# YessionCC/AR-NeRF

Measured on AMD Instinct MI355X. Metric: training rays/sec + test PSNR, Lego 8192-ray batch, 1/2/4/8 MI355X, higher is better.
Workload: dtype fp16 field (MLP forward, backward and weight gradients on fp16 MFMA operands, fp32 accumulate) / fp32 march, composite, Adam; 1 GPU; lego-shaped training step: 8192 rays/rank, scale 0.5, 1 x 128^3 grid, L=16 F=2 T=2^19 hash, 64-wide MLPs, raw loss, Adam lr 1e-2; batch_rays_per_gpu=8192, global_batch_rays=8192, pretrain_steps=2000, graphs=True, chunk_first=64, row_forward=1, march_fork=r1, parallelism=dp1, hash_backward=hybrid, bin_level_lo=8, bin_merge_hi=11, steps_per_graph_replay=2, erode=False

## Files before the change

### ar-nerf_amd/csrc/field.hip

```cpp
#pragma clang fp contract(off)

#include <algorithm>

#include "common.h"
#include "field_net.h"
#include "grid.h"
#include "transmittance.h"

namespace ngp {

struct __attribute__((aligned(4))) u2a4 {
    uint32_t x, y;
    __device__ operator uint2() const { return make_uint2(x, y); }
};

__device__ __forceinline__ uint32_t pick4(uint4 q, uint32_t k) {
    return k == 0 ? q.x : k == 1 ? q.y : k == 2 ? q.z : q.w;
}

__device__ __forceinline__ void fetch_pair(const uint32_t* __restrict__ tl, uint32_t i0, uint32_t i1, bool dense,
                                           uint32_t& v0, uint32_t& v1) {
    const uint32_t lo = min(i0, i1), hi = max(i0, i1);
    uint32_t vlo, vhi;
    if (dense) {
// ... 90 lines not shown
    uint32_t pg[3];
    level_cell(in, u, pg, pos);
    gather_cell(pg, u, table, v);
}
__device__ __forceinline__ uint32_t level_sum_h2(const float in[3], const LevelU& u, const uint32_t v[8]) {
    float pos[3], w[8];
    uint32_t pg[3];
    level_cell(in, u, pg, pos);
    corner_weights(pos, w);
    float a0, a1;
    sum_level(w, v, a0, a1);
    return pack_h2(a0, a1);
}

__device__ __forceinline__ void encode_level(const float in[3], const LevelU& u, const uint32_t* __restrict__ table,
                                             float& a0, float& a1) {
    float pos[3], w[8];
    uint32_t pg[3], v[8];
    level_cell(in, u, pg, pos);
    corner_weights(pos, w);
#pragma unroll
    for (int yz = 0; yz < 4; ++yz) {
        uint32_t i0, i1;
        pair_index(pg, yz, u, i0, i1);
        fetch_pair(table + u.off, i0, i1, u.dense || !u.pow2, v[2 * yz], v[2 * yz + 1]);
    }
    sum_level(w, v, a0, a1);
}

__device__ __forceinline__ h8 encode4(const float in[3], int g, const LevelLds& lv, const uint32_t* __restrict__ table) {
    h8 e;
#pragma unroll
    for (int jl = 0; jl < 4; ++jl) {
        float a0, a1;
        encode_level(in, level_lane(lv, 4 * g + jl), table, a0, a1);
        e[2 * jl] = (_Float16)a0;
        e[2 * jl + 1] = (_Float16)a1;
    }
    return e;
}


template <bool COLOR, bool ENC_IN = false>
__global__ void __launch_bounds__(256) field_fwd_kernel(const float* __restrict__ xyzs, const float* __restrict__ dirs,
                                                        int64_t n, const int64_t* __restrict__ n_dev, GridArgs ga,
                                                        const uint32_t* __restrict__ table,
                                                        const _Float16* __restrict__ mlp, float* __restrict__ sigmas,
                                                        float* __restrict__ rgbs, _Float16* __restrict__ enc_out,
                                                        _Float16* __restrict__ h_out,
                                                        const _Float16* __restrict__ enc_in = nullptr,
                                                        int64_t enc_stride = 0,
                                                        const int32_t* __restrict__ sidx = nullptr,
                                                        int act = NGP_RGB_SIGMOID) {
    __shared__ __attribute__((aligned(16))) _Float16 sw[SWF];
    __shared__ LevelLds lv;
    load_fwd_weights_direct(mlp, sw, COLOR);
    if constexpr (!ENC_IN) load_levels(ga, lv);
    __syncthreads();
    const int64_t N = ngp_capped_count(n_dev, n);
    const int lane = threadIdx.x & 63, s = lane & 15, g = lane >> 4;
    const int64_t nw = (int64_t)gridDim.x * (blockDim.x >> 6);
    for (int64_t base = ((int64_t)blockIdx.x * (blockDim.x >> 6) + (threadIdx.x >> 6)) * 16; base < N; base += nw * 16) {
        const int64_t j = base + s;
        const bool valid = j < N;
        const int64_t i = valid && sidx ? (int64_t)sidx[j] : j;
        h8 e;
        if constexpr (ENC_IN) {
            const h4 z4 = {0, 0, 0, 0};
            const h4 ea = valid ? *reinterpret_cast<const h4*>(enc_in + ((2 * g) * enc_stride + i) * 4) : z4;
            const h4 eb = valid ? *reinterpret_cast<const h4*>(enc_in + ((2 * g + 1) * enc_stride + i) * 4) : z4;
            e = pack(ea, eb);
        } else {
            float in[3];
            load_x01(xyzs, i, valid, ga, in);
            e = encode4(in, g, lv, table);
        }
        h4 h1[4];
        const h4 hh = density_net(e, sw, s, g, h1);
        if (valid) {
            if (enc_out) *reinterpret_cast<h8*>(enc_out + i * 32 + 8 * g) = e;
            if (h_out) *reinterpret_cast<h4*>(h_out + i * 16 + 4 * g) = hh;
            if (g == 0) sigmas[i] = expf((float)hh[0]);
        }
        if constexpr (COLOR) {
            const float dx = valid ? dirs[3 * i] : 0.f, dy = valid ? dirs[3 * i + 1] : 0.f,
                        dz = valid ? dirs[3 * i + 2] : 1.f;
            float sh[4];
            sh4_select(dx, dy, dz, g, sh);
            const h8 cin = {(_Float16)sh[0], (_Float16)sh[1], (_Float16)sh[2], (_Float16)sh[3], hh[0], hh[1], hh[2], hh[3]};
            h4 h3[4], h4v[4];
            const h4 o = color_net(cin, sw, s, g, h3, h4v);
            if (valid && g == 0) {
                rgbs[3 * i] = rgb_out(o[0], act);
                rgbs[3 * i + 1] = rgb_out(o[1], act);
                rgbs[3 * i + 2] = rgb_out(o[2], act);
            }
        }
    }
}

__global__ void __launch_bounds__(256) hash_encode_kernel(const float* __restrict__ xyzs, int64_t n,
                                                          const int64_t* __restrict__ n_dev,
                                                          const int32_t* __restrict__ sidx, GridArgs ga,
                                                          const uint32_t* __restrict__ table,
                                                          _Float16* __restrict__ enc_pm) {
    __shared__ LevelLds lv;
    load_levels(ga, lv);
    __syncthreads();
    const int64_t N = ngp_capped_count(n_dev, n);
    for (int64_t j = (int64_t)blockIdx.x * blockDim.x + threadIdx.x; j < N; j += (int64_t)gridDim.x * blockDim.x) {
        const int64_t i = sidx ? (int64_t)sidx[j] : j;
        float in[3];
        load_x01(xyzs, i, true, ga, in);
#pragma unroll 1
        for (int pr = 0; pr < 8; ++pr) {
            float w[2][8];
            uint32_t v[2][8];
            gather_level_u(in, level_u(lv, 2 * pr), table, w[0], v[0]);
            gather_level_u(in, level_u(lv, 2 * pr + 1), table, w[1], v[1]);
            float a0, a1, b0, b1;
            sum_level(w[0], v[0], a0, a1);
            sum_level(w[1], v[1], b0, b1);
            *reinterpret_cast<h4*>(enc_pm + ((int64_t)pr * n + i) * 4) =
                h4{(_Float16)a0, (_Float16)a1, (_Float16)b0, (_Float16)b1};
        }
    }
}

__device__ __forceinline__ void transpose_rows4(uint32_t E[16]) {
#pragma unroll
    for (int k = 0; k < 4; ++k) {
        const auto a = __builtin_amdgcn_permlane32_swap(E[k], E[8 + k], false, false);
        E[k] = a[0];
        E[8 + k] = a[1];
        const auto b = __builtin_amdgcn_permlane32_swap(E[4 + k], E[12 + k], false, false);
        E[4 + k] = b[0];
        E[12 + k] = b[1];
    }
#pragma unroll
    for (int k = 0; k < 4; ++k) {
        const auto a = __builtin_amdgcn_permlane16_swap(E[k], E[4 + k], false, false);
        E[k] = a[0];
        E[4 + k] = a[1];
        const auto b = __builtin_amdgcn_permlane16_swap(E[8 + k], E[12 + k], false, false);
        E[8 + k] = b[0];
        E[12 + k] = b[1];
    }
}

constexpr int FEM2_WAVES = 8, FEM_LPR = 2;
constexpr int PRE_LEVELS = 8;
static_assert(PRE_LEVELS % FEM_LPR == 0 && PRE_LEVELS % 2 == 0, "pre-encoded levels: whole rounds and pairs");
static_assert(L % FEM_LPR == 0, "levels per round");
__device__ __forceinline__ void encode_rounds(const float in[3], const LevelLds& lv, const uint32_t* __restrict__ table,
                                              int r0, uint32_t E[16]) {
#pragma unroll 1
    for (int r = r0; r < L / FEM_LPR; ++r) {
        uint32_t v[FEM_LPR][8];
#pragma unroll
        for (int q = 0; q < FEM_LPR; ++q) gather_level_loads(in, level_u(lv, FEM_LPR * r + q), table, v[q]);
#pragma unroll
        for (int q = 0; q < 16 - FEM_LPR; ++q) E[q] = E[q + FEM_LPR];
#pragma unroll
        for (int q = 0; q < FEM_LPR; ++q) E[16 - FEM_LPR + q] = level_sum_h2(in, level_u(lv, FEM_LPR * r + q), v[q]);
    }
}
template <bool COLOR>
__global__ void __launch_bounds__(64 * FEM2_WAVES, FEM2_WAVES / 2) field_encode_mlp_reg_kernel(
    const float* __restrict__ xyzs, const float* __restrict__ dirs, int64_t n, const int64_t* __restrict__ n_dev,
    const int32_t* __restrict__ sidx, GridArgs ga, const uint32_t* __restrict__ table,
    const _Float16* __restrict__ mlp, _Float16* __restrict__ enc_pm, float* __restrict__ sigmas,
    float* __restrict__ rgbs, _Float16* __restrict__ h_out, int act) {
    __shared__ __attribute__((aligned(16))) _Float16 sw[SWF];
    __shared__ LevelLds lv;
    NGP_PROBE_BEGIN(NGP_P_FIELD_ENCODE_MLP);
    const int64_t N = ngp_capped_count(n_dev, n);
    const int lane = threadIdx.x & 63, wv = threadIdx.x >> 6;
    const int64_t G = gridDim.x;
    const int64_t chunks = (N + 63) >> 6;
    int64_t k = (int64_t)wv * G + blockIdx.x;
    int64_t i_first = 0;
    float in_first[3];
    {
        const int64_t j = k * 64 + lane;
        const bool valid = k < chunks && j < N;
        i_first = valid ? (sidx ? (int64_t)sidx[j] : j) : 0;
        load_x01(xyzs, i_first, valid, ga, in_first);
    }
    load_fwd_weights_direct(mlp, sw, COLOR);
    load_levels(ga, lv);
    __syncthreads();
    bool first = true;
    for (; k < chunks; k += (int64_t)FEM2_WAVES * G) {
        int lane_l = lane;
        asm volatile("" : "+v"(lane_l));
        const int s = lane_l & 15, g = lane_l >> 4;
        const int64_t j = k * 64 + lane_l;
        const bool valid = j < N;
        int64_t i = i_first;
        float in[3] = {in_first[0], in_first[1], in_first[2]};
        if (!first) {
            i = valid ? (sidx ? (int64_t)sidx[j] : j) : 0;
            load_x01(xyzs, i, valid, ga, in);
        }
        first = false;
        uint32_t E[16];
        encode_rounds(in, lv, table, 0, E);
        if (valid && enc_pm) {
#pragma unroll
            for (int pr = 0; pr < 8; ++pr)
                *reinterpret_cast<uint2*>(enc_pm + ((int64_t)pr * n + i) * 4) = make_uint2(E[2 * pr], E[2 * pr + 1]);
        }
        transpose_rows4(E);
        const int32_t imine = valid ? (int32_t)i : -1;
#pragma unroll 1
        for (int c = 0; c < 4; ++c) {
            const int32_t ic = __shfl(imine, 16 * c + s, 64);
            const bool ok = ic >= 0;
            const h8 e = __builtin_bit_cast(h8, make_uint4(E[0], E[1], E[2], E[3]));
#pragma unroll
            for (int q = 0; q < 12; ++q) E[q] = E[q + 4];
            h4 h1[4];
            const h4 hh = density_net(e, sw, s, g, h1);
            if (ok) {
                if (h_out) *reinterpret_cast<h4*>(h_out + (int64_t)ic * 16 + 4 * g) = hh;
                if (g == 0) sigmas[ic] = expf((float)hh[0]);
            }
            if constexpr (COLOR) {
                const float dx = ok ? dirs[3 * (int64_t)ic] : 0.f, dy = ok ? dirs[3 * (int64_t)ic + 1] : 0.f,
                            dz = ok ? dirs[3 * (int64_t)ic + 2] : 1.f;
                float sh[4];
                sh4_select(dx, dy, dz, g, sh);
                const h8 cin = {(_Float16)sh[0], (_Float16)sh[1], (_Float16)sh[2], (_Float16)sh[3], hh[0], hh[1], hh[2], hh[3]};
                h4 h3[4], h4v[4];
                const h4 o = color_net(cin, sw, s, g, h3, h4v);
                if (ok && g == 0) {
                    rgbs[3 * (int64_t)ic] = rgb_out(o[0], act);
                    rgbs[3 * (int64_t)ic + 1] = rgb_out(o[1], act);
                    rgbs[3 * (int64_t)ic + 2] = rgb_out(o[2], act);
                }
            }
        }
    }
    NGP_PROBE_END();
}

template <bool COLOR>
__device__ __forceinline__ float encode_mlp_chunk(const float* __restrict__ xyzs, const float* __restrict__ dirs,
                                                  int64_t i0, int cnt, int64_t n, const GridArgs& ga,
                                                  const LevelLds& lv, const uint32_t* __restrict__ table,
                                                  const _Float16* sw, _Float16* __restrict__ enc_pm,
                                                  float* __restrict__ sigmas, float* __restrict__ rgbs, int pre = 0,
                                                  int act = NGP_RGB_SIGMOID) {
    int lane_l = threadIdx.x & 63;
    asm volatile("" : "+v"(lane_l));
    const int s = lane_l & 15, g = lane_l >> 4;
    const bool valid = lane_l < cnt;
    const int64_t i = i0 + lane_l;
    float in[3];
    load_x01(xyzs, i, valid, ga, in);
    uint32_t E[16];
    if (pre) {
#pragma unroll
        for (int pr = 0; pr < PRE_LEVELS / 2; ++pr) {
            const uint2 q = valid ? *reinterpret_cast<const uint2*>(enc_pm + ((int64_t)pr * n + i) * 4) : make_uint2(0u, 0u);
            E[16 - PRE_LEVELS + 2 * pr] = q.x;
            E[16 - PRE_LEVELS + 2 * pr + 1] = q.y;
        }
    }
    encode_rounds(in, lv, table, pre / FEM_LPR, E);
    if (valid && enc_pm) {
#pragma unroll
        for (int pr = 0; pr < 8; ++pr)
            if (2 * pr >= pre)
                *reinterpret_cast<uint2*>(enc_pm + ((int64_t)pr * n + i) * 4) = make_uint2(E[2 * pr], E[2 * pr + 1]);
    }
    transpose_rows4(E);
    float sg = 0.f;
#pragma unroll 1
    for (int c = 0; c < 4; ++c) {
        if (16 * c >= cnt) break;
        const bool ok = 16 * c + s < cnt;
        const int64_t ic = i0 + 16 * c + s;
        const h8 e = __builtin_bit_cast(h8, make_uint4(E[0], E[1], E[2], E[3]));
#pragma unroll
        for (int q = 0; q < 12; ++q) E[q] = E[q + 4];
        h4 h1[4];
        const h4 hh = density_net(e, sw, s, g, h1);
        const float sig = expf((float)hh[0]);
        if (ok && g == 0) sigmas[ic] = sig;
        const float sgc = __shfl(sig, lane_l & 15, 64);
        if ((lane_l >> 4) == c) sg = sgc;
        if constexpr (COLOR) {
            const float dx = ok ? dirs[3 * ic] : 0.f, dy = ok ? dirs[3 * ic + 1] : 0.f, dz = ok ? dirs[3 * ic + 2] : 1.f;
            float sh[4];
            sh4_select(dx, dy, dz, g, sh);
            const h8 cin = {(_Float16)sh[0], (_Float16)sh[1], (_Float16)sh[2], (_Float16)sh[3], hh[0], hh[1], hh[2], hh[3]};
            h4 h3[4], h4v[4];
            const h4 o = color_net(cin, sw, s, g, h3, h4v);
            if (ok && g == 0) {
                rgbs[3 * ic] = rgb_out(o[0], act);
                rgbs[3 * ic + 1] = rgb_out(o[1], act);
                rgbs[3 * ic + 2] = rgb_out(o[2], act);
            }
        }
    }
    return sg;
}

template <bool COLOR>
__global__ void __launch_bounds__(64 * FEM2_WAVES, FEM2_WAVES / 2) field_first_chunk_kernel(
    const float* __restrict__ xyzs, const float* __restrict__ dirs, const float* __restrict__ deltas,
    const int64_t* __restrict__ rays_a, const int32_t* __restrict__ rows, const int64_t* __restrict__ n_rows_dev,
    int64_t n_rows, int64_t n, float T_thr, GridArgs ga, const uint32_t* __restrict__ table,
    const _Float16* __restrict__ mlp, _Float16* __restrict__ enc_pm, float* __restrict__ sigmas,
    float* __restrict__ rgbs, int32_t* __restrict__ rest, int32_t* __restrict__ list2, int64_t* __restrict__ total2,
    int64_t* __restrict__ evaluated, int pre, int act) {
    __shared__ __attribute__((aligned(16))) _Float16 sw[SWF];
    __shared__ LevelLds lv;
    __shared__ unsigned long long blk_eval;
    NGP_PROBE_BEGIN(NGP_P_FIRST_CHUNK);
    const int lane = threadIdx.x & 63, wv = threadIdx.x >> 6;
    const int64_t NR = ngp_capped_count(n_rows_dev, n_rows);
    const int64_t G = gridDim.x, stride = (int64_t)FEM2_WAVES * G;
    int64_t j = (int64_t)wv * G + blockIdx.x;
    int64_t r = 0, start = 0, N = 0;
    if (j < NR) {
        r = rows ? (int64_t)rows[j] : j;
        start = rays_a[3 * r + 1];
        N = rays_a[3 * r + 2];
    }
    if (threadIdx.x == 0) blk_eval = 0ull;
    load_fwd_weights_direct(mlp, sw, COLOR);
    load_levels(ga, lv);
    __syncthreads();
    int64_t ev = 0;
    for (; j < NR; j += stride) {
        const int cnt = (int)(N < 64 ? N : 64);
        int32_t rc = 0;
        if (cnt > 0) {
            const float dl = lane < cnt ? deltas[start + lane] : 0.f;
            const float sg = encode_mlp_chunk<COLOR>(xyzs, dirs, start, cnt, n, ga, lv, table, sw, enc_pm, sigmas, rgbs,
                                                     pre, act);
            const float om = 1.0f - (1.0f - __expf(-sg * dl));
            const ChunkT ct = chunk_transmittance(om, cnt, 1.0f, T_thr, lane);
            rc = (!ct.hit && N > 64) ? (int32_t)(N - 64) : 0;
            ev += cnt;
        }
        if (rest && lane == 0) rest[r] = rc;
        if (list2 && rc > 0) {
            unsigned long long o = 0;
            if (lane == 0) o = atomicAdd((unsigned long long*)total2, (unsigned long long)rc);
            const int64_t o2 = (int64_t)__shfl(o, 0, 64);
            if (lane == 0 && o2 + rc > n) ngp_guard_hit();
            for (int t = lane; t < rc && o2 + t < n; t += 64) list2[o2 + t] = (int32_t)(start + 64 + t);
            ev += rc;
        }
        const int64_t jn = j + stride;
        if (jn < NR) {
            r = rows ? (int64_t)rows[jn] : jn;
            start = rays_a[3 * r + 1];
            N = rays_a[3 * r + 2];
        }
    }
    if (lane == 0 && ev) atomicAdd(&blk_eval, (unsigned long long)ev);
    __syncthreads();
    if (threadIdx.x == 0 && evaluated && blk_eval) atomicAdd((unsigned long long*)evaluated, blk_eval);
    NGP_PROBE_END();
}

__global__ void __launch_bounds__(256) encode_coarse_first_kernel(
    const float* __restrict__ xyzs, const int64_t* __restrict__ rays_a, const int32_t* __restrict__ rows,
    const int64_t* __restrict__ n_rows_dev, int64_t n_rows, int64_t n, GridArgs ga,
    const uint32_t* __restrict__ table, _Float16* __restrict__ enc_pm) {
    __shared__ LevelLds lv;
    NGP_PROBE_BEGIN(NGP_P_PRE_ENCODE);
    load_levels(ga, lv);
    __syncthreads();
    const int lane = threadIdx.x & 63;
    const int64_t NR = ngp_capped_count(n_rows_dev, n_rows);
    constexpr int NP = PRE_LEVELS / 2;
    const int64_t stride = (int64_t)gridDim.x * (blockDim.x >> 6);
    for (int64_t q = (int64_t)blockIdx.x * (blockDim.x >> 6) + (threadIdx.x >> 6); q < NR * NP; q += stride) {
        const int64_t j = q / NP;
        const int pr = (int)(q - j * NP);
        const int64_t r = rows ? (int64_t)rows[j] : j;
        const int64_t start = rays_a[3 * r + 1], N = rays_a[3 * r + 2];
        const bool valid = lane < N;
        const int64_t i = start + lane;
        float in[3];
        load_x01(xyzs, i, valid, ga, in);
        uint32_t v[2][8];
        gather_level_loads(in, level_u(lv, 2 * pr), table, v[0]);
        gather_level_loads(in, level_u(lv, 2 * pr + 1), table, v[1]);
        const uint32_t e0 = level_sum_h2(in, level_u(lv, 2 * pr), v[0]);
        const uint32_t e1 = level_sum_h2(in, level_u(lv, 2 * pr + 1), v[1]);
        if (valid) *reinterpret_cast<uint2*>(enc_pm + ((int64_t)pr * n + i) * 4) = make_uint2(e0, e1);
    }
    NGP_PROBE_END();
}

__device__ __forceinline__ void coarse_level_runs(const float in[3], bool valid, float gd, int l, const LevelLds& lv,
                                                  int lane, int cx, uint32_t idx[4], float v[4], uint64_t heads[4]) {
    const float sc = lv.scale[l];
    const uint32_t res = lv.res[l], size = lv.size[l], off = lv.off[l];
    const bool dense = (lv.dense >> l) & 1u, pow2 = (lv.pow2 >> l) & 1u;
    float pos[3];
    uint32_t pg[3];
    level_cell(sc, in, pg, pos);
#pragma unroll
    for (int yz = 0; yz < 4; ++yz) {
        const int cy = yz & 1, cz = yz >> 1;
        float wt = 1.0f;
        wt *= cx ? pos[0] : 1 - pos[0];
        wt *= cy ? pos[1] : 1 - pos[1];
        wt *= cz ? pos[2] : 1 - pos[2];
        idx[yz] = valid ? off + corner_index(pg[0] + cx, pg[1] + cy, pg[2] + cz, res, size, dense, pow2)
                        : 0xffffffffu;
        v[yz] = wt * gd;
    }
    uint32_t prev[4];
#pragma unroll
    for (int yz = 0; yz < 4; ++yz) prev[yz] = __shfl_up(idx[yz], 4, 64);
#pragma unroll
    for (int yz = 0; yz < 4; ++yz) heads[yz] = __ballot(lane < 4 || prev[yz] != idx[yz]);
    if ((heads[0] & heads[1] & heads[2] & heads[3]) != ~0ull) {
#pragma unroll
        for (int o4 = 4; o4 < 64; o4 <<= 1) {
            float ov[4];
#pragma unroll
            for (int yz = 0; yz < 4; ++yz) ov[yz] = __shfl_down(v[yz], o4, 64);
            const uint64_t span = ((0x1111111111111111ull & ((2ull << o4) - 1ull)) & ~1ull) << lane;
#pragma unroll
            for (int yz = 0; yz < 4; ++yz)
                if (lane + o4 < 64 && (heads[yz] & span) == 0) v[yz] += ov[yz];
        }
    }
}

__device__ __forceinline__ void coarse_scatter_level(const float in[3], bool valid, float gd, int l, const LevelLds& lv,
                                                     float* __restrict__ dst, int lane, int cx, int f) {
    uint32_t idx[4];
    float v[4];
    uint64_t heads[4];
    coarse_level_runs(in, valid, gd, l, lv, lane, cx, idx, v, heads);
#pragma unroll
    for (int yz = 0; yz < 4; ++yz) {
        const bool head = (heads[yz] >> lane) & 1ull;
        if (head && valid) atomicAdd(&dst[2 * (size_t)idx[yz] + f], v[yz]);
    }
}

typedef _Float16 h2v __attribute__((ext_vector_type(2)));
__device__ __forceinline__ f4 mfma16(h4 a, h4 b, f4 c) { return __builtin_amdgcn_mfma_f32_16x16x16f16(a, b, c, 0, 0, 0); }
__device__ __forceinline__ h4 lds4(const _Float16* p) { return *reinterpret_cast<const h4*>(p); }

constexpr int RT16 = 20, RT64 = 68;
constexpr int BT5 = SWF, BT4 = BT5 + 64 * RT16, BT3 = BT4 + 64 * RT64, BT2 = BT3 + 16 * RT64, BT1 = BT2 + 64 * RT16,
              BTE = BT1 + 32 * RT64;
constexpr int TROW = 16, TTILE = 16 * TROW;
constexpr int SCR = (BTE + 7) & ~7;

__device__ __forceinline__ void load_bwd_weights(const _Float16* __restrict__ mlp, _Float16* sw) {
    const int t = threadIdx.x, nt = blockDim.x;
    for (int e = t; e < 64 * 16; e += nt) { const int i = e >> 4, o = e & 15; sw[BT5 + i * RT16 + o] = mlp[OW5 + o * 64 + i]; }
    for (int e = t; e < 64 * 64; e += nt) { const int i = e >> 6, o = e & 63; sw[BT4 + i * RT64 + o] = mlp[OW4 + o * 64 + i]; }
    for (int e = t; e < 16 * 64; e += nt) { const int i = e >> 6, o = e & 63; sw[BT3 + i * RT64 + o] = mlp[OW3 + o * 32 + 16 + i]; }
    for (int e = t; e < 64 * 16; e += nt) { const int i = e >> 4, o = e & 15; sw[BT2 + i * RT16 + o] = mlp[OW2 + o * 64 + i]; }
    for (int e = t; e < 32 * 64; e += nt) { const int i = e >> 6, o = e & 63; sw[BT1 + i * RT64 + o] = mlp[OW1 + o * 32 + i]; }
}

__device__ __forceinline__ void load_bwd_weights_direct(const _Float16* __restrict__ mlp, _Float16* sw) {
    constexpr int N1 = 128, N2 = 64, N3 = 128, N4 = 256, N5 = 64, NI = N1 + N2 + N3 + N4 + N5;
    for (int it = threadIdx.x; it < NI; it += blockDim.x) {
        int ow, lg_cb, li, bt, rt, skip;
        if (it < N1) { ow = OW1; lg_cb = 2; li = it; bt = BT1; rt = RT64; skip = 0; }
        else if (it < N1 + N2) { ow = OW2; lg_cb = 3; li = it - N1; bt = BT2; rt = RT16; skip = 0; }
        else if (it < N1 + N2 + N3) { ow = OW3; lg_cb = 2; li = it - N1 - N2; bt = BT3; rt = RT64; skip = 16; }
        else if (it < NI - N5) { ow = OW4; lg_cb = 3; li = it - N1 - N2 - N3; bt = BT4; rt = RT64; skip = 0; }
        else { ow = OW5; lg_cb = 3; li = it - (NI - N5); bt = BT5; rt = RT16; skip = 0; }
        const int in_dim = 8 << lg_cb, o = 2 * (li >> lg_cb), i0 = 8 * (li & ((1 << lg_cb) - 1));
        const int f0 = ow + o * in_dim + i0;
        const h8 a = *reinterpret_cast<const h8*>(mlp + f0);
        const h8 b = *reinterpret_cast<const h8*>(mlp + f0 + in_dim);
        place_fwd8(f0, a, sw);
        place_fwd8(f0 + in_dim, b, sw);
        if (i0 >= skip) {
#pragma unroll
            for (int jj = 0; jj < 8; ++jj)
                *reinterpret_cast<h2v*>(sw + bt + (i0 - skip + jj) * rt + o) = h2v{a[jj], b[jj]};
        }
    }
}

__device__ __forceinline__ float max4(f4 v) { return fmaxf(fmaxf(fabsf(v[0]), fabsf(v[1])), fmaxf(fabsf(v[2]), fabsf(v[3]))); }
constexpr int E_MIN = -100, E_MAX = 100;
__device__ __forceinline__ int fexp(float m) { return (int)(__float_as_uint(m) >> 23) - 126; }
__device__ __forceinline__ int next_exp(float m_scaled, int e_prev) {
    return min(max(e_prev + 14 - fexp(m_scaled), E_MIN), E_MAX);
}
__device__ __forceinline__ h4 cvt4(f4 v, float r) {
    return h4{(_Float16)(v[0] * r), (_Float16)(v[1] * r), (_Float16)(v[2] * r), (_Float16)(v[3] * r)};
}
__device__ __forceinline__ uint32_t mask_h2(uint32_t gv, uint32_t av) {
    const s16x2 t = __builtin_bit_cast(s16x2, __builtin_bit_cast(u16x2, av) + (u16x2){0x7fff, 0x7fff});
    return gv & __builtin_bit_cast(uint32_t, t >> (s16x2){15, 15});
}
__device__ __forceinline__ h4 relu_mask(h4 gr, h4 act) {
    const uint2 gv = __builtin_bit_cast(uint2, gr), av = __builtin_bit_cast(uint2, act);
// ... 449 lines not shown
        dirs, n, n_dev, sample_idx, (const _Float16*)enc_f16, (const _Float16*)mlp_f16, dL_dsigmas, dL_drgbs, denc_ws,
        grad_mlp, enc_pm_stride, act));
    return ngp_launch_status();
}

}

using namespace ngp;

extern "C" {

#define NGP_CHECK_RGB_ACT(a) NGP_CHECK_ARG((a) >= NGP_RGB_SIGMOID && (a) <= NGP_RGB_RELU)

int ngp_field_forward(const float* xyzs, const float* dirs, int64_t n, const int64_t* n_dev,
                      const ngp_hashgrid_t* grid, const void* table_f16, const void* mlp_f16, float* sigmas,
                      float* rgbs, void* enc_f16, void* h_f16, void* stream) {
    return ngp_field_forward_act(xyzs, dirs, n, n_dev, grid, table_f16, mlp_f16, sigmas, rgbs, enc_f16, h_f16,
                                 NGP_RGB_SIGMOID, stream);
}

int ngp_field_forward_act(const float* xyzs, const float* dirs, int64_t n, const int64_t* n_dev,
                          const ngp_hashgrid_t* grid, const void* table_f16, const void* mlp_f16, float* sigmas,
                          float* rgbs, void* enc_f16, void* h_f16, int rgb_act, void* stream) {
    NGP_CHECK_RGB_ACT(rgb_act);
    GridArgs ga;
    int st = grid_args(grid, ga);
    if (st) return st;
    NGP_CHECK_ARG(n >= 0);
    if (n == 0) return NGP_OK;
    NGP_CHECK_ARG(xyzs && dirs && table_f16 && mlp_f16 && sigmas && rgbs);
    NGP_CHECK_ARG(((uintptr_t)table_f16 & 15) == 0);
    NGP_CHECK_ARG(((uintptr_t)mlp_f16 & 15) == 0);
    static const unsigned cap = resident_blocks(field_fwd_kernel<true>, 256, 0);
    field_fwd_kernel<true><<<persistent_blocks(n, 64, cap), 256, 0, as_stream(stream)>>>(
        xyzs, dirs, n, n_dev, ga, (const uint32_t*)table_f16, (const _Float16*)mlp_f16, sigmas, rgbs,
        (_Float16*)enc_f16, (_Float16*)h_f16, nullptr, 0, nullptr, rgb_act);
    return ngp_launch_status();
}

int ngp_field_forward_indexed(const float* xyzs, const float* dirs, int64_t n, const int64_t* n_dev,
                              const int32_t* sample_idx, const ngp_hashgrid_t* grid, const void* table_f16,
                              const void* mlp_f16, float* sigmas, float* rgbs, void* enc_f16, void* stream) {
    GridArgs ga;
    int st = grid_args(grid, ga);
    if (st) return st;
    NGP_CHECK_ARG(n >= 0);
    if (n == 0) return NGP_OK;
    NGP_CHECK_ARG(xyzs && dirs && sample_idx && table_f16 && mlp_f16 && sigmas && rgbs);
    NGP_CHECK_ARG(((uintptr_t)table_f16 & 15) == 0);
    NGP_CHECK_ARG(((uintptr_t)mlp_f16 & 15) == 0);
    static const unsigned cap = resident_blocks(field_fwd_kernel<true>, 256, 0);
    field_fwd_kernel<true><<<persistent_blocks(n, 64, cap), 256, 0, as_stream(stream)>>>(
        xyzs, dirs, n, n_dev, ga, (const uint32_t*)table_f16, (const _Float16*)mlp_f16, sigmas, rgbs,
        (_Float16*)enc_f16, nullptr, nullptr, 0, sample_idx);
    return ngp_launch_status();
}

int ngp_density_forward(const float* xyzs, int64_t n, const int64_t* n_dev, const ngp_hashgrid_t* grid,
                        const void* table_f16, const void* mlp_f16, float* sigmas, void* h_f16, void* stream) {
    GridArgs ga;
    int st = grid_args(grid, ga);
    if (st) return st;
    NGP_CHECK_ARG(n >= 0);
    if (n == 0) return NGP_OK;
    NGP_CHECK_ARG(xyzs && table_f16 && mlp_f16 && sigmas);
    NGP_CHECK_ARG(((uintptr_t)table_f16 & 15) == 0);
    NGP_CHECK_ARG(((uintptr_t)mlp_f16 & 15) == 0);
    static const unsigned cap = resident_blocks(field_fwd_kernel<false>, 256, 0);
    field_fwd_kernel<false><<<persistent_blocks(n, 64, cap), 256, 0, as_stream(stream)>>>(
        xyzs, nullptr, n, n_dev, ga, (const uint32_t*)table_f16, (const _Float16*)mlp_f16, sigmas, nullptr, nullptr,
        (_Float16*)h_f16);
    return ngp_launch_status();
}

int ngp_hash_encode(const float* xyzs, int64_t n, const int64_t* n_dev, const int32_t* sample_idx,
                    const ngp_hashgrid_t* grid, const void* table_f16, void* enc_pm, void* stream) {
    GridArgs ga;
    int st = grid_args(grid, ga);
    if (st) return st;
    NGP_CHECK_ARG(n >= 0);
    if (n == 0) return NGP_OK;
    NGP_CHECK_ARG(xyzs && table_f16 && enc_pm && ((uintptr_t)enc_pm & 7) == 0);
    NGP_CHECK_ARG(((uintptr_t)table_f16 & 15) == 0);
    hipStream_t s = as_stream(stream);
    static const unsigned cap = resident_blocks(hash_encode_kernel, 256, 0);
    NGP_TIMED(NGP_K_HASH_ENCODE, s, hash_encode_kernel<<<std::max(1u, std::min(cap, (unsigned)((n + 255) / 256))), 256, 0, s>>>(
        xyzs, n, n_dev, sample_idx, ga, (const uint32_t*)table_f16, (_Float16*)enc_pm));
    return ngp_launch_status();
}

int ngp_field_encode_mlp(const float* xyzs, const float* dirs, int64_t n, const int64_t* n_dev,
                         const int32_t* sample_idx, const ngp_hashgrid_t* grid, const void* table_f16,
                         const void* mlp_f16, void* enc_pm, float* sigmas, float* rgbs, void* h_f16, void* stream) {
    return ngp_field_encode_mlp_act(xyzs, dirs, n, n_dev, sample_idx, grid, table_f16, mlp_f16, enc_pm, sigmas, rgbs,
                                    h_f16, NGP_RGB_SIGMOID, stream);
}

int ngp_field_encode_mlp_act(const float* xyzs, const float* dirs, int64_t n, const int64_t* n_dev,
                             const int32_t* sample_idx, const ngp_hashgrid_t* grid, const void* table_f16,
                             const void* mlp_f16, void* enc_pm, float* sigmas, float* rgbs, void* h_f16, int rgb_act,
                             void* stream) {
    NGP_CHECK_RGB_ACT(rgb_act);
    GridArgs ga;
    int st = grid_args(grid, ga);
    if (st) return st;
    NGP_CHECK_ARG(n >= 0);
    if (n == 0) return NGP_OK;
    NGP_CHECK_ARG(xyzs && table_f16 && mlp_f16 && sigmas && (dirs != nullptr) == (rgbs != nullptr));
    NGP_CHECK_ARG(((uintptr_t)table_f16 & 15) == 0 && ((uintptr_t)mlp_f16 & 15) == 0 && ((uintptr_t)enc_pm & 7) == 0);
    hipStream_t s = as_stream(stream);
    if (!dirs) {
        static const unsigned capd = resident_blocks(field_encode_mlp_reg_kernel<false>, 64 * FEM2_WAVES, 0);
        NGP_TIMED(NGP_K_HASH_ENCODE, s, field_encode_mlp_reg_kernel<false><<<std::max(1u, std::min(capd, (unsigned)((n + 64 * FEM2_WAVES - 1) / (64 * FEM2_WAVES)))), 64 * FEM2_WAVES, 0, s>>>(
            xyzs, nullptr, n, n_dev, sample_idx, ga, (const uint32_t*)table_f16, (const _Float16*)mlp_f16,
            (_Float16*)enc_pm, sigmas, nullptr, (_Float16*)h_f16, NGP_RGB_SIGMOID));
        return ngp_launch_status();
    }
    static const unsigned capr = resident_blocks(field_encode_mlp_reg_kernel<true>, 64 * FEM2_WAVES, 0);
    NGP_TIMED(NGP_K_HASH_ENCODE, s, field_encode_mlp_reg_kernel<true><<<std::max(1u, std::min(capr, (unsigned)((n + 64 * FEM2_WAVES - 1) / (64 * FEM2_WAVES)))), 64 * FEM2_WAVES, 0, s>>>(
        xyzs, dirs, n, n_dev, sample_idx, ga, (const uint32_t*)table_f16, (const _Float16*)mlp_f16,
        (_Float16*)enc_pm, sigmas, rgbs, (_Float16*)h_f16, rgb_act));
    return ngp_launch_status();
}

int ngp_field_forward_first_pre(const float* xyzs, const float* dirs, const float* deltas, const int64_t* rays_a,
                                const int32_t* rows, const int64_t* n_rows_dev, int64_t n_rows, int64_t n,
                                float T_threshold, const ngp_hashgrid_t* grid, const void* table_f16,
                                const void* mlp_f16, void* enc_pm, float* sigmas, float* rgbs, int32_t* rest,
                                int32_t* list2, int64_t* total2, int64_t* evaluated, int pre_levels, void* stream) {
    return ngp_field_forward_first_pre_act(xyzs, dirs, deltas, rays_a, rows, n_rows_dev, n_rows, n, T_threshold, grid,
                                           table_f16, mlp_f16, enc_pm, sigmas, rgbs, rest, list2, total2, evaluated,
                                           pre_levels, NGP_RGB_SIGMOID, stream);
}

int ngp_field_forward_first_pre_act(const float* xyzs, const float* dirs, const float* deltas, const int64_t* rays_a,
                                    const int32_t* rows, const int64_t* n_rows_dev, int64_t n_rows, int64_t n,
                                    float T_threshold, const ngp_hashgrid_t* grid, const void* table_f16,
                                    const void* mlp_f16, void* enc_pm, float* sigmas, float* rgbs, int32_t* rest,
                                    int32_t* list2, int64_t* total2, int64_t* evaluated, int pre_levels, int rgb_act,
                                    void* stream) {
    NGP_CHECK_RGB_ACT(rgb_act);
    NGP_CHECK_ARG(pre_levels == 0 || (pre_levels == PRE_LEVELS && enc_pm));
    GridArgs ga;
    int st = grid_args(grid, ga);
    if (st) return st;
    NGP_CHECK_ARG(n_rows >= 0 && n >= 0);
    if (n_rows == 0) return NGP_OK;
    NGP_CHECK_ARG(xyzs && dirs && deltas && rays_a && table_f16 && mlp_f16 && sigmas && rgbs && (rest || list2));
    NGP_CHECK_ARG(!list2 || (total2 && ((uintptr_t)total2 & 7) == 0));
    NGP_CHECK_ARG(((uintptr_t)table_f16 & 15) == 0 && ((uintptr_t)mlp_f16 & 15) == 0 && ((uintptr_t)enc_pm & 7) == 0 &&
                  ((uintptr_t)evaluated & 7) == 0);
    hipStream_t s = as_stream(stream);
    static const unsigned cap = resident_blocks(field_first_chunk_kernel<true>, 64 * FEM2_WAVES, 0);
    const unsigned blocks = std::max(1u, std::min(cap, (unsigned)((n_rows + FEM2_WAVES - 1) / FEM2_WAVES)));
    NGP_TIMED(NGP_K_HASH_ENCODE, s, field_first_chunk_kernel<true><<<blocks, 64 * FEM2_WAVES, 0, s>>>(
        xyzs, dirs, deltas, rays_a, rows, n_rows_dev, n_rows, n, T_threshold, ga, (const uint32_t*)table_f16,
        (const _Float16*)mlp_f16, (_Float16*)enc_pm, sigmas, rgbs, rest, list2, total2, evaluated, pre_levels,
        rgb_act));
    return ngp_launch_status();
}

int ngp_field_forward_first(const float* xyzs, const float* dirs, const float* deltas, const int64_t* rays_a,
                            const int32_t* rows, const int64_t* n_rows_dev, int64_t n_rows, int64_t n,
                            float T_threshold, const ngp_hashgrid_t* grid, const void* table_f16, const void* mlp_f16,
                            void* enc_pm, float* sigmas, float* rgbs, int32_t* rest, int32_t* list2,
                            int64_t* total2, int64_t* evaluated, void* stream) {
    return ngp_field_forward_first_pre(xyzs, dirs, deltas, rays_a, rows, n_rows_dev, n_rows, n, T_threshold, grid,
                                       table_f16, mlp_f16, enc_pm, sigmas, rgbs, rest, list2, total2, evaluated, 0,
                                       stream);
}

int ngp_field_encode_first_coarse(const float* xyzs, const int64_t* rays_a, const int32_t* rows,
                                  const int64_t* n_rows_dev, int64_t n_rows, int64_t n, const ngp_hashgrid_t* grid,
                                  const void* table_f16, void* enc_pm, void* stream) {
    GridArgs ga;
    int st = grid_args(grid, ga);
    if (st) return st;
    NGP_CHECK_ARG(n_rows >= 0 && n >= 0);
    if (n_rows == 0) return NGP_OK;
    NGP_CHECK_ARG(xyzs && rays_a && table_f16 && enc_pm && ((uintptr_t)table_f16 & 15) == 0 &&
                  ((uintptr_t)enc_pm & 7) == 0);
    hipStream_t s = as_stream(stream);
    static const unsigned cap = resident_blocks(encode_coarse_first_kernel, 256, 0);
    const unsigned blocks = std::max(1u, std::min(cap, (unsigned)((n_rows * (PRE_LEVELS / 2) + 3) / 4)));
    encode_coarse_first_kernel<<<blocks, 256, 0, s>>>(xyzs, rays_a, rows, n_rows_dev, n_rows, n, ga,
                                                      (const uint32_t*)table_f16, (_Float16*)enc_pm);
    return ngp_launch_status();
}

int ngp_field_mlp_forward(const void* enc_pm, const float* dirs, int64_t n, const int64_t* n_dev,
                          const int32_t* sample_idx, const void* mlp_f16, float* sigmas, float* rgbs, void* h_f16,
                          void* stream) {
    NGP_CHECK_ARG(n >= 0);
    if (n == 0) return NGP_OK;
    NGP_CHECK_ARG(enc_pm && mlp_f16 && sigmas && (dirs != nullptr) == (rgbs != nullptr));
    NGP_CHECK_ARG(((uintptr_t)mlp_f16 & 15) == 0 && ((uintptr_t)enc_pm & 7) == 0);
    GridArgs ga{};
    if (!dirs) {
        static const unsigned capd = resident_blocks(field_fwd_kernel<false, true>, 256, 0);
        NGP_TIMED(NGP_K_FIELD_MLP, as_stream(stream),
                  field_fwd_kernel<false, true><<<persistent_blocks(n, 64, capd), 256, 0, as_stream(stream)>>>(
                      nullptr, nullptr, n, n_dev, ga, nullptr, (const _Float16*)mlp_f16, sigmas, nullptr, nullptr,
                      (_Float16*)h_f16, (const _Float16*)enc_pm, n, sample_idx));
        return ngp_launch_status();
    }
    static const unsigned cap = resident_blocks(field_fwd_kernel<true, true>, 256, 0);
    NGP_TIMED(NGP_K_FIELD_MLP, as_stream(stream),
              field_fwd_kernel<true, true><<<persistent_blocks(n, 64, cap), 256, 0, as_stream(stream)>>>(
                  nullptr, dirs, n, n_dev, ga, nullptr, (const _Float16*)mlp_f16, sigmas, rgbs, nullptr,
                  (_Float16*)h_f16, (const _Float16*)enc_pm, n, sample_idx));
    return ngp_launch_status();
}

int ngp_field_backward_mlp(const float* dirs, int64_t n, const int64_t* n_dev, const int32_t* sample_idx,
                           const void* enc_f16, int64_t enc_pm_stride, const void* mlp_f16, const float* dL_dsigmas,
                           const float* dL_drgbs, float* denc_ws, float* grad_mlp, void* stream) {
    return ngp_field_backward_mlp_act(dirs, n, n_dev, sample_idx, enc_f16, enc_pm_stride, mlp_f16, dL_dsigmas,
                                      dL_drgbs, denc_ws, grad_mlp, NGP_RGB_SIGMOID, stream);
}

int ngp_field_backward_mlp_act(const float* dirs, int64_t n, const int64_t* n_dev, const int32_t* sample_idx,
                               const void* enc_f16, int64_t enc_pm_stride, const void* mlp_f16,
                               const float* dL_dsigmas, const float* dL_drgbs, float* denc_ws, float* grad_mlp,
                               int rgb_act, void* stream) {
    NGP_CHECK_RGB_ACT(rgb_act);
    NGP_CHECK_ARG(n >= 0);
    if (n == 0) return NGP_OK;
    NGP_CHECK_ARG(dirs && enc_f16 && mlp_f16 && dL_dsigmas && dL_drgbs && denc_ws && grad_mlp);
    NGP_CHECK_ARG(((uintptr_t)mlp_f16 & 15) == 0);
    return launch_bwd_mlp(dirs, n, n_dev, sample_idx, enc_f16, enc_pm_stride, mlp_f16, dL_dsigmas, dL_drgbs,
                          denc_ws, grad_mlp, rgb_act, stream);
}

int ngp_hash_backward(const float* xyzs, int64_t n, const int64_t* n_dev, const int32_t* sample_idx,
                      const ngp_hashgrid_t* grid, const float* denc, float* grad_table, void* stream) {
    GridArgs ga;
    int st = grid_args(grid, ga);
    if (st) return st;
    NGP_CHECK_ARG(n >= 0);
    if (n == 0) return NGP_OK;
    NGP_CHECK_ARG(xyzs && denc && grad_table && ((uintptr_t)denc & 15) == 0);
    NGP_TIMED(NGP_K_HASH_BWD_COARSE, as_stream(stream), hash_bwd_kernel<<<persistent_blocks(n, 64, HASH_BWD_BLOCKS), 256, 0, as_stream(stream)>>>(xyzs, n, n_dev, sample_idx,
                                                                                     ga, denc, grad_table, 0, L));
    return ngp_launch_status();
}

}

static void launch_coarse(const float* xyzs, int64_t n, const int64_t* n_dev, const int32_t* sample_idx,
                          const GridArgs& ga, const float* denc, float* grad_table, int lo, int hi, float* rep,
                          int rep_hi, uint32_t rep_stride, int nrep, hipStream_t s) {
    NGP_TIMED(NGP_K_HASH_BWD_COARSE, s, hash_bwd_kernel<<<persistent_blocks(n, 64, COARSE_BLOCKS), 256, 0, s>>>(
        xyzs, n, n_dev, sample_idx, ga, denc, grad_table, lo, hi, rep, rep_hi, rep_stride, nrep));
}

extern "C" {

int ngp_hash_backward_levels(const float* xyzs, int64_t n, const int64_t* n_dev, const int32_t* sample_idx,
                             const ngp_hashgrid_t* grid, const float* denc, float* grad_table, int level_lo,
                             int level_hi, void* stream) {
    GridArgs ga;
    int st = grid_args(grid, ga);
    if (st) return st;
    NGP_CHECK_ARG(n >= 0 && 0 <= level_lo && level_lo <= level_hi && level_hi <= L);
    if (n == 0 || level_lo == level_hi) return NGP_OK;
    NGP_CHECK_ARG(xyzs && denc && grad_table && ((uintptr_t)denc & 15) == 0);
    launch_coarse(xyzs, n, n_dev, sample_idx, ga, denc, grad_table, level_lo, level_hi, nullptr, 0, 0, 1,
                  as_stream(stream));
    return ngp_launch_status();
}

int ngp_hash_backward_levels_rep(const float* xyzs, int64_t n, const int64_t* n_dev, const int32_t* sample_idx,
                                 const ngp_hashgrid_t* grid, const float* denc, float* grad_table, int level_lo,
                                 int level_hi, float* rep, int rep_levels, int n_rep, int fold, void* stream) {
    GridArgs ga;
    int st = grid_args(grid, ga);
    if (st) return st;
    NGP_CHECK_ARG(n >= 0 && 0 <= level_lo && level_lo <= level_hi && level_hi <= L);
    NGP_CHECK_ARG(0 <= rep_levels && rep_levels <= level_hi && n_rep >= 1 && n_rep <= 64);
    if (rep_levels == 0 || !rep)
        return ngp_hash_backward_levels(xyzs, n, n_dev, sample_idx, grid, denc, grad_table, level_lo, level_hi,
                                        stream);
    if (n == 0 || level_lo == level_hi) return NGP_OK;
    NGP_CHECK_ARG(xyzs && denc && grad_table && ((uintptr_t)denc & 15) == 0);
    NGP_CHECK_ARG(((uintptr_t)grad_table & 15) == 0 && ((uintptr_t)rep & 15) == 0);
    const uint32_t nfl = 2u * grid->offsets[rep_levels];
    NGP_CHECK_ARG(nfl % 4 == 0);
    hipStream_t s = as_stream(stream);
    launch_coarse(xyzs, n, n_dev, sample_idx, ga, denc, grad_table, level_lo, level_hi, rep, rep_levels, nfl, n_rep, s);
    if (!fold) return ngp_launch_status();
    const uint32_t n4 = nfl / 4;
    const unsigned rb = std::min(2048u, (n4 + 255) / 256);
    if (n_rep <= 8)
        NGP_TIMED(NGP_K_HASH_BWD_COARSE, s, rep_reduce_kernel<8><<<rb, 256, 0, s>>>(grad_table, rep, n4, n4, n_rep));
    else if (n_rep <= 16)
        NGP_TIMED(NGP_K_HASH_BWD_COARSE, s, rep_reduce_kernel<16><<<rb, 256, 0, s>>>(grad_table, rep, n4, n4, n_rep));
    else
        NGP_TIMED(NGP_K_HASH_BWD_COARSE, s, rep_reduce_kernel<64><<<rb, 256, 0, s>>>(grad_table, rep, n4, n4, n_rep));
    return ngp_launch_status();
}

size_t ngp_hash_backward_rep_floats(const ngp_hashgrid_t* grid, int rep_levels, int n_rep) {
    if (!grid || rep_levels < 0 || rep_levels > L || n_rep < 1) return 0;
    return (size_t)n_rep * 2u * grid->offsets[rep_levels];
}

int ngp_field_backward(const float* xyzs, const float* dirs, int64_t n, const int64_t* n_dev,
// ... 23 lines not shown
```

Measured before the change: 19.07 million rays/s.

## Split first-chunk encode and MLP across wave pairs sharing LDS

```diff
diff --git a/ar-nerf_amd/csrc/field.hip b/ar-nerf_amd/csrc/field.hip
--- a/ar-nerf_amd/csrc/field.hip
+++ b/ar-nerf_amd/csrc/field.hip
@@ -266,17 +266,21 @@
 constexpr int PRE_LEVELS = 8;
 static_assert(PRE_LEVELS % FEM_LPR == 0 && PRE_LEVELS % 2 == 0, "pre-encoded levels: whole rounds and pairs");
 static_assert(L % FEM_LPR == 0, "levels per round");
+constexpr int FIRST_LPR = 2;
+static_assert((PRE_LEVELS / 2) % FIRST_LPR == 0 && ((L - PRE_LEVELS) / 2) % FIRST_LPR == 0 && (L / 2) % FIRST_LPR == 0,
+              "a wave's half of the levels: whole rounds");
+template <int LPR, int NE>
 __device__ __forceinline__ void encode_rounds(const float in[3], const LevelLds& lv, const uint32_t* __restrict__ table,
-                                              int r0, uint32_t E[16]) {
+                                              int r0, int r1, uint32_t (&E)[NE]) {
 #pragma unroll 1
-    for (int r = r0; r < L / FEM_LPR; ++r) {
-        uint32_t v[FEM_LPR][8];
-#pragma unroll
-        for (int q = 0; q < FEM_LPR; ++q) gather_level_loads(in, level_u(lv, FEM_LPR * r + q), table, v[q]);
-#pragma unroll
-        for (int q = 0; q < 16 - FEM_LPR; ++q) E[q] = E[q + FEM_LPR];
-#pragma unroll
-        for (int q = 0; q < FEM_LPR; ++q) E[16 - FEM_LPR + q] = level_sum_h2(in, level_u(lv, FEM_LPR * r + q), v[q]);
+    for (int r = r0; r < r1; ++r) {
+        uint32_t v[LPR][8];
+#pragma unroll
+        for (int q = 0; q < LPR; ++q) gather_level_loads(in, level_u(lv, LPR * r + q), table, v[q]);
+#pragma unroll
+        for (int q = 0; q < NE - LPR; ++q) E[q] = E[q + LPR];
+#pragma unroll
+        for (int q = 0; q < LPR; ++q) E[NE - LPR + q] = level_sum_h2(in, level_u(lv, LPR * r + q), v[q]);
     }
 }
 template <bool COLOR>
@@ -319,7 +323,7 @@
         }
         first = false;
         uint32_t E[16];
-        encode_rounds(in, lv, table, 0, E);
+        encode_rounds<FEM_LPR>(in, lv, table, 0, L / FEM_LPR, E);
         if (valid && enc_pm) {
 #pragma unroll
             for (int pr = 0; pr < 8; ++pr)
@@ -359,46 +363,60 @@
     NGP_PROBE_END();
 }
 
-template <bool COLOR>
-__device__ __forceinline__ float encode_mlp_chunk(const float* __restrict__ xyzs, const float* __restrict__ dirs,
-                                                  int64_t i0, int cnt, int64_t n, const GridArgs& ga,
-                                                  const LevelLds& lv, const uint32_t* __restrict__ table,
-                                                  const _Float16* sw, _Float16* __restrict__ enc_pm,
-                                                  float* __restrict__ sigmas, float* __restrict__ rgbs, int pre = 0,
-                                                  int act = NGP_RGB_SIGMOID) {
+constexpr int FC_PAIRS = FEM2_WAVES / 2;
+struct __attribute__((aligned(16))) PairLds {
+    uint32_t enc[4][64][4];
+    float sg[32];
+};
+
+__device__ __forceinline__ void encode_half_chunk(const float* __restrict__ xyzs, int64_t i0, int cnt, int64_t n,
+                                                  const GridArgs& ga, const LevelLds& lv,
+                                                  const uint32_t* __restrict__ table, _Float16* __restrict__ enc_pm,
+                                                  PairLds& P, int half, int pre) {
     int lane_l = threadIdx.x & 63;
     asm volatile("" : "+v"(lane_l));
-    const int s = lane_l & 15, g = lane_l >> 4;
     const bool valid = lane_l < cnt;
     const int64_t i = i0 + lane_l;
     float in[3];
     load_x01(xyzs, i, valid, ga, in);
-    uint32_t E[16];
+    const int ng = (L - pre) / 2, l0 = pre + half * ng;
+    uint32_t H[8];
     if (pre) {
 #pragma unroll
-        for (int pr = 0; pr < PRE_LEVELS / 2; ++pr) {
+        for (int t = 0; t < PRE_LEVELS / 4; ++t) {
+            const int pr = half * (PRE_LEVELS / 4) + t;
             const uint2 q = valid ? *reinterpret_cast<const uint2*>(enc_pm + ((int64_t)pr * n + i) * 4) : make_uint2(0u, 0u);
-            E[16 - PRE_LEVELS + 2 * pr] = q.x;
-            E[16 - PRE_LEVELS + 2 * pr + 1] = q.y;
-        }
-    }
-    encode_rounds(in, lv, table, pre / FEM_LPR, E);
+            H[8 - PRE_LEVELS / 2 + 2 * t] = q.x;
+            H[8 - PRE_LEVELS / 2 + 2 * t + 1] = q.y;
+        }
+    }
+    encode_rounds<FIRST_LPR>(in, lv, table, l0 / FIRST_LPR, (l0 + ng) / FIRST_LPR, H);
     if (valid && enc_pm) {
 #pragma unroll
-        for (int pr = 0; pr < 8; ++pr)
-            if (2 * pr >= pre)
-                *reinterpret_cast<uint2*>(enc_pm + ((int64_t)pr * n + i) * 4) = make_uint2(E[2 * pr], E[2 * pr + 1]);
-    }
-    transpose_rows4(E);
+        for (int t = 0; t < 4; ++t)
+            if (2 * t >= 8 - ng)
+                *reinterpret_cast<uint2*>(enc_pm + ((int64_t)((l0 + 2 * t - (8 - ng)) / 2) * n + i) * 4) =
+                    make_uint2(H[2 * t], H[2 * t + 1]);
+    }
+    const int q0 = pre ? half : 2 * half, q1 = pre ? 2 + half : 2 * half + 1;
+    *reinterpret_cast<uint4*>(P.enc[q0][lane_l]) = make_uint4(H[0], H[1], H[2], H[3]);
+    *reinterpret_cast<uint4*>(P.enc[q1][lane_l]) = make_uint4(H[4], H[5], H[6], H[7]);
+}
+
+template <bool COLOR>
+__device__ __forceinline__ float mlp_half_chunk(const float* __restrict__ dirs, int64_t i0, int cnt, const PairLds& P,
+                                                int half, const _Float16* sw, float* __restrict__ sigmas,
+                                                float* __restrict__ rgbs, int act) {
+    int lane_l = threadIdx.x & 63;
+    asm volatile("" : "+v"(lane_l));
+    const int s = lane_l & 15, g = lane_l >> 4;
     float sg = 0.f;
 #pragma unroll 1
-    for (int c = 0; c < 4; ++c) {
+    for (int c = 2 * half; c < 2 * half + 2; ++c) {
         if (16 * c >= cnt) break;
         const bool ok = 16 * c + s < cnt;
         const int64_t ic = i0 + 16 * c + s;
-        const h8 e = __builtin_bit_cast(h8, make_uint4(E[0], E[1], E[2], E[3]));
-#pragma unroll
-        for (int q = 0; q < 12; ++q) E[q] = E[q + 4];
+        const h8 e = __builtin_bit_cast(h8, *reinterpret_cast<const uint4*>(P.enc[g][16 * c + s]));
         h4 h1[4];
         const h4 hh = density_net(e, sw, s, g, h1);
         const float sig = expf((float)hh[0]);
@@ -423,7 +441,7 @@
 }
 
 template <bool COLOR>
-__global__ void __launch_bounds__(64 * FEM2_WAVES, FEM2_WAVES / 2) field_first_chunk_kernel(
+__global__ void __launch_bounds__(64 * FEM2_WAVES, 6) field_first_chunk_kernel(
     const float* __restrict__ xyzs, const float* __restrict__ dirs, const float* __restrict__ deltas,
     const int64_t* __restrict__ rays_a, const int32_t* __restrict__ rows, const int64_t* __restrict__ n_rows_dev,
     int64_t n_rows, int64_t n, float T_thr, GridArgs ga, const uint32_t* __restrict__ table,
@@ -432,12 +450,15 @@
     int64_t* __restrict__ evaluated, int pre, int act) {
     __shared__ __attribute__((aligned(16))) _Float16 sw[SWF];
     __shared__ LevelLds lv;
+    __shared__ PairLds pairs[FC_PAIRS];
     __shared__ unsigned long long blk_eval;
     NGP_PROBE_BEGIN(NGP_P_FIRST_CHUNK);
-    const int lane = threadIdx.x & 63, wv = threadIdx.x >> 6;
+    const int lane = threadIdx.x & 63, wv = (int)rfl(threadIdx.x >> 6), half = wv & 1;
+    PairLds& P = pairs[wv >> 1];
     const int64_t NR = ngp_capped_count(n_rows_dev, n_rows);
-    const int64_t G = gridDim.x, stride = (int64_t)FEM2_WAVES * G;
-    int64_t j = (int64_t)wv * G + blockIdx.x;
+    const int64_t G = gridDim.x, stride = (int64_t)FC_PAIRS * G;
+    int64_t jb = blockIdx.x;
+    int64_t j = (int64_t)(wv >> 1) * G + jb;
     int64_t r = 0, start = 0, N = 0;
     if (j < NR) {
         r = rows ? (int64_t)rows[j] : j;
@@ -449,26 +470,37 @@
     load_levels(ga, lv);
     __syncthreads();
     int64_t ev = 0;
-    for (; j < NR; j += stride) {
-        const int cnt = (int)(N < 64 ? N : 64);
-        int32_t rc = 0;
+    for (; jb < NR; jb += stride, j += stride) {
+        const bool have = j < NR;
+        const int cnt = have ? (int)(N < 64 ? N : 64) : 0;
+        float dl = 0.f;
         if (cnt > 0) {
-            const float dl = lane < cnt ? deltas[start + lane] : 0.f;
-            const float sg = encode_mlp_chunk<COLOR>(xyzs, dirs, start, cnt, n, ga, lv, table, sw, enc_pm, sigmas, rgbs,
-                                                     pre, act);
-            const float om = 1.0f - (1.0f - __expf(-sg * dl));
-            const ChunkT ct = chunk_transmittance(om, cnt, 1.0f, T_thr, lane);
-            rc = (!ct.hit && N > 64) ? (int32_t)(N - 64) : 0;
-            ev += cnt;
-        }
-        if (rest && lane == 0) rest[r] = rc;
-        if (list2 && rc > 0) {
-            unsigned long long o = 0;
-            if (lane == 0) o = atomicAdd((unsigned long long*)total2, (unsigned long long)rc);
-            const int64_t o2 = (int64_t)__shfl(o, 0, 64);
-            if (lane == 0 && o2 + rc > n) ngp_guard_hit();
-            for (int t = lane; t < rc && o2 + t < n; t += 64) list2[o2 + t] = (int32_t)(start + 64 + t);
-            ev += rc;
+            if (!half && lane < cnt) dl = deltas[start + lane];
+            encode_half_chunk(xyzs, start, cnt, n, ga, lv, table, enc_pm, P, half, pre);
+        }
+        __syncthreads();
+        float sg = 0.f;
+        if (cnt > 32 * half) sg = mlp_half_chunk<COLOR>(dirs, start, cnt, P, half, sw, sigmas, rgbs, act);
+        if (half && lane >= 32) P.sg[lane - 32] = sg;
+        __syncthreads();
+        if (have && !half) {
+            int32_t rc = 0;
+            if (cnt > 0) {
+                if (lane >= 32) sg = P.sg[lane - 32];
+                const float om = 1.0f - (1.0f - __expf(-sg * dl));
+                const ChunkT ct = chunk_transmittance(om, cnt, 1.0f, T_thr, lane);
+                rc = (!ct.hit && N > 64) ? (int32_t)(N - 64) : 0;
+                ev += cnt;
+            }
+            if (rest && lane == 0) rest[r] = rc;
+            if (list2 && rc > 0) {
+                unsigned long long o = 0;
+                if (lane == 0) o = atomicAdd((unsigned long long*)total2, (unsigned long long)rc);
+                const int64_t o2 = (int64_t)__shfl(o, 0, 64);
+                if (lane == 0 && o2 + rc > n) ngp_guard_hit();
+                for (int t = lane; t < rc && o2 + t < n; t += 64) list2[o2 + t] = (int32_t)(start + 64 + t);
+                ev += rc;
+            }
         }
         const int64_t jn = j + stride;
         if (jn < NR) {
@@ -1224,7 +1256,7 @@
                   ((uintptr_t)evaluated & 7) == 0);
     hipStream_t s = as_stream(stream);
     static const unsigned cap = resident_blocks(field_first_chunk_kernel<true>, 64 * FEM2_WAVES, 0);
-    const unsigned blocks = std::max(1u, std::min(cap, (unsigned)((n_rows + FEM2_WAVES - 1) / FEM2_WAVES)));
+    const unsigned blocks = std::max(1u, std::min(cap, (unsigned)((n_rows + FC_PAIRS - 1) / FC_PAIRS)));
     NGP_TIMED(NGP_K_HASH_ENCODE, s, field_first_chunk_kernel<true><<<blocks, 64 * FEM2_WAVES, 0, s>>>(
         xyzs, dirs, deltas, rays_a, rows, n_rows_dev, n_rows, n, T_threshold, ga, (const uint32_t*)table_f16,
         (const _Float16*)mlp_f16, (_Float16*)enc_pm, sigmas, rgbs, rest, list2, total2, evaluated, pre_levels,
```

Result: no change. 19.16 million rays/s (median of 3 runs) (+0.4%).
